# Xharlie/BtcDet

Hardware: AMD Instinct MI355X
Metric: scenes/s fwd+bwd KITTI-Car bs=2/GPU (BtcDet hot path) (higher is better)
Workload: dtype f32

## Files before the change

btcdet_amd/_lib.py:

```python
import ctypes
import os

import numpy as np
import torch

_HERE = os.path.dirname(os.path.abspath(__file__))
LIB_PATH = os.path.join(_HERE, "libbtcdet_hip.so")
_lib = None

c_i32p = ctypes.POINTER(ctypes.c_int32)
c_f32p = ctypes.POINTER(ctypes.c_float)
vp = ctypes.c_void_p
ci = ctypes.c_int
sz = ctypes.c_size_t

MODE_SUBM, MODE_CONV, MODE_TRANSPOSE = 0, 1, 2


class BtcHipError(RuntimeError):
    pass


class BtcOccConfig(ctypes.Structure):
    _fields_ = [("batch", ctypes.c_int32), ("grid", ctypes.c_int32 * 3), ("sphere_grid", ctypes.c_int32 * 3),
# ... 102 lines not shown
    "btc_revoxelize_fill": (ci, [vp, vp, ci, ci, ci, c_i32p, ci, ci, vp, vp, vp, vp, sz, vp]),
    "btc_pass_occ_vox_ws_bytes": (sz, [ctypes.POINTER(BtcPovConfig), ci, ci]),
    "btc_pass_occ_vox_count": (ci, [ctypes.POINTER(BtcPovConfig), vp, vp, vp, vp, vp, vp, ci, ci, ci, vp, vp, sz, vp]),
    "btc_pass_occ_vox_fill": (ci, [ctypes.POINTER(BtcPovConfig), vp, ci, ci, ci, ci, ci, ci, vp, vp, vp, vp, vp, vp, sz, vp]),
    "btc_pass_occ_vox_fill_i32": (ci, [ctypes.POINTER(BtcPovConfig), vp, ci, ci, ci, ci, ci, ci, vp, vp, vp, vp, vp, vp, vp, vp, sz, vp]),
    "btc_occ_loss_ws_bytes": (sz, []),
    "btc_occ_loss_fwd": (ci, [vp, vp, vp, vp, vp, vp, vp, vp, ci, ctypes.c_longlong, ctypes.c_float, ctypes.c_float, ctypes.c_float, vp, vp, vp,
                              sz, vp]),
    "btc_occ_loss_bwd": (ci, [vp, vp, vp, vp, vp, vp, vp, vp, ci, ctypes.c_longlong, ctypes.c_float, vp, vp, vp, vp, vp]),
    "btc_occ_loss_fwd_total": (ci, [vp, vp, vp, vp, vp, vp, vp, vp, ci, ctypes.c_longlong, ctypes.c_float, ctypes.c_float, ctypes.c_float, vp, vp,
                                    vp, sz, vp]),
    "btc_occ_loss_bwd_total": (ci, [vp, vp, vp, vp, vp, vp, vp, vp, ci, ctypes.c_longlong, ctypes.c_float, vp, vp, vp, vp, vp]),
    "btc_dense_split_fwd": (ci, [vp, vp, ci, ci, ci, vp, vp, vp, vp]),
    "btc_occ_prob": (ci, [vp, vp, ci, ctypes.c_longlong, vp, vp]),
    "btc_dense_split_bwd": (ci, [vp, vp, vp, ci, ci, ci, vp, vp, vp]),
    "btc_cat_pad_fwd": (ci, [vp, ci, vp, ci, ctypes.c_longlong, ci, ci, vp, vp]),
    "btc_cat_pad_bwd": (ci, [vp, ci, ctypes.c_longlong, ci, vp, ci, vp, ci, vp]),
    "btc_sumsq2_ws_bytes": (sz, []),
    "btc_sumsq2_fwd": (ci, [vp, ctypes.c_longlong, ci, ctypes.c_double, vp, ctypes.c_longlong, ci, ctypes.c_double, vp, vp, sz, vp]),
    "btc_sumsq2_bwd": (ci, [vp, ctypes.c_longlong, ci, ctypes.c_float, vp, vp, ctypes.c_longlong, ci, ctypes.c_float, vp, vp, vp]),
    "btc_bn_ws_bytes": (sz, [ci]),
    "btc_bn_relu_fwd": (ci, [vp, ci, ci, vp, vp, vp, vp, vp, ctypes.c_float, ctypes.c_float, ci, ci, vp, vp, vp, vp, sz, vp]),
    "btc_spin": (ci, [ci, vp]),
    "btc_bn_relu_bwd": (ci, [vp, vp, vp, ci, ci, vp, vp, vp, ci, ci, vp, vp, vp, vp, sz, vp]),
    "btc_bn_relu_fwd_bf16": (ci, [vp, ci, ci, vp, vp, vp, vp, vp, ctypes.c_float, ctypes.c_float, ci, ci, vp, vp, vp, vp, sz, vp]),
    "btc_bn_relu_bwd_bf16": (ci, [vp, vp, vp, ci, ci, vp, vp, vp, ci, ci, vp, vp, vp, vp, sz, vp]),
    "btc_ball_query": (ci, [vp, vp, vp, vp, ci, ci, ctypes.c_float, ctypes.c_float, ci, vp, vp]),
    "btc_group_points": (ci, [vp, vp, vp, vp, ci, ci, ci, ci, vp, vp]),
    "btc_group_points_grad": (ci, [vp, vp, vp, vp, ci, ci, ci, ci, ci, vp, vp]),
    "btc_furthest_point_sampling": (ci, [vp, ci, ci, ci, vp, vp, vp]),
    "btc_three_nn": (ci, [vp, vp, vp, vp, ci, ci, vp, vp, vp]),
    "btc_three_interpolate": (ci, [vp, vp, vp, ci, ci, vp, vp]),
    "btc_three_interpolate_grad": (ci, [vp, vp, vp, ci, ci, ci, vp, vp]),
    "btc_bn_fuse_ws_bytes": (sz, []),
    "btc_conv_bn_relu_fwd": (ci, [ci, vp, vp, vp, vp, vp, ci, ci, ci, ci, vp, vp, vp, vp, vp, vp, ctypes.c_float, ctypes.c_float, ci, vp, vp, vp, vp, sz, vp, vp]),
    "btc_conv_bn_relu_fwd_src": (ci, [ci, vp, ctypes.c_longlong, vp, vp, vp, vp, ci, ci, ci, ci, vp, vp, vp, vp, vp, vp, ctypes.c_float, ctypes.c_float, ci, vp, vp, vp, vp, sz, vp, vp]),
    "btc_col_sum": (ci, [vp, ci, ci, vp, vp, sz, vp]),
    "btc_col_sum_bf16": (ci, [vp, ci, ci, vp, vp, sz, vp]),
    "btc_occ_targets_ws_bytes": (sz, [ctypes.POINTER(BtcOccConfig)]),
    "btc_occ_backproject_lut": (ci, [ctypes.POINTER(BtcOccConfig), vp, vp]),
    "btc_occ_targets": (ci, [ctypes.POINTER(BtcOccConfig), vp, vp, vp, ci, ci, ci, vp, vp, vp, vp, ci, vp, vp,
                             ctypes.POINTER(BtcOccBuffers), vp, sz, vp]),
}

EXPORTED_SYMBOLS = tuple(_SIGS.keys())

_INFER_SIGS = {
    "btc_conv_bn_eval_fwd": (ci, [ci, vp, ctypes.c_longlong, vp, vp, vp, vp, ci, ci, ci, ci, vp, vp, vp, vp, ctypes.c_float, ci, vp, vp]),
    "btc_det_select_nms_ws_bytes": (sz, [ci, ci]),
    "btc_det_select_nms": (ci, [vp, vp, ci, ci, ci, ci, ci, ctypes.c_float, ctypes.c_float, ci, ci, ci, vp, vp, vp, vp, sz, vp]),
    "btc_det_finish": (ci, [vp, vp, ci, ci, ci, ci, ci, ci, vp, vp, vp, vp, ci, vp, ci, ci, vp, ci, ci, c_f32p, ci, vp, vp, vp, vp, vp, vp]),
    "btc_occ_metrics_ws_bytes": (sz, [ci, ci]),
    "btc_occ_metrics": (ci, [vp, vp, vp, vp, ctypes.c_longlong, vp, vp, vp, ctypes.c_longlong, vp, vp, ci, ci, ci, vp, vp, sz, vp]),
    "btc_kitti_overlaps": (ci, [vp, vp, vp, vp, vp, c_i32p, ci, vp, vp, vp]),
    "btc_kitti_match_tp": (ci, [vp, vp, vp, vp, vp, vp, vp, c_i32p, ci, ci, ci, ci, ci, ci, vp, vp, vp]),
    "btc_kitti_match_stats_ws_bytes": (sz, [ci, ci, ci, ci, ci]),
    "btc_kitti_match_stats": (ci, [vp, vp, vp, vp, vp, vp, vp, vp, vp, vp, vp, c_i32p, ci, ci, ci, ci, ci, ci, ci, vp, vp, vp, sz, vp]),
}

INFER_EXPORTED_SYMBOLS = tuple(_INFER_SIGS.keys())

_AUGMENT_SIGS = {
    "btc_augment_ws_bytes": (sz, [ci, ci, ci]),
    "btc_augment_batch": (ci, [vp, ci, ci, vp, ci, vp, vp, vp, ctypes.c_longlong, vp, vp, vp, vp, ci, ctypes.c_longlong, vp, vp,
                               ctypes.c_longlong, vp, vp, vp, vp, sz, vp]),
    "btc_world_transform": (ci, [vp, ci, ci, vp, ci, vp, vp, vp, vp]),
}

AUGMENT_EXPORTED_SYMBOLS = tuple(_AUGMENT_SIGS.keys())

_BESTMATCH_SIGS = {
    "btc_place_templates": (ci, [vp, ctypes.c_longlong, vp, vp, vp, vp, vp, ci, ci, vp, vp, ctypes.c_longlong, ci, vp, vp]),
}

BESTMATCH_EXPORTED_SYMBOLS = tuple(_BESTMATCH_SIGS.keys())

_FRAMES_SIGS = {
    "btc_fov_crop_ws_bytes": (sz, [ci, ci]),
    "btc_fov_crop": (ci, [vp, ci, ci, vp, ci, vp, ci, vp, vp, vp, vp, sz, vp]),
}

FRAMES_EXPORTED_SYMBOLS = tuple(_FRAMES_SIGS.keys())


def lib():
    global _lib
    if _lib is None:
        if not os.path.exists(LIB_PATH):
            raise BtcHipError(
                f"{LIB_PATH} not found: build it with `python -c 'import __graft_entry__ as g; g.build()'` "
                f"or `make -C btcdet_amd/csrc` (there is no CPU fallback for the hot path)")
        L = ctypes.CDLL(LIB_PATH)
        for name, (res, args) in (list(_SIGS.items()) + list(_INFER_SIGS.items()) + list(_AUGMENT_SIGS.items()) + list(_BESTMATCH_SIGS.items()) +
                                  list(_FRAMES_SIGS.items())):
            fn = getattr(L, name)
            fn.restype = res
            fn.argtypes = args
        for kv in filter(None, os.environ.get("BTC_TUNE", "").split(",")):
            k, v = kv.split("=")
            if L.btc_tune_set(int(k), int(v)) != 0:
                raise BtcHipError("BTC_TUNE: bad entry %r" % kv)
        _lib = L
    return _lib


_fast = False


def fast():
    global _fast
    if _fast is False:
        _fast = None
        if os.environ.get("BTC_FASTPATH", "1") != "0":
            try:
                lib()
                from . import _btcfast
                if _btcfast.abi_version() == lib().btc_version():
                    _fast = _btcfast
            except ImportError:
                _fast = None
    return _fast


def check(rc, what):
    if rc != 0:
        msg = lib().btc_last_error().decode("utf-8", "replace")
        raise BtcHipError(f"{what} failed (code {rc}): {msg}")


_raw_stream = torch._C._cuda_getCurrentRawStream
_cur_device = torch._C._cuda_getDevice


def stream_ptr():
    return _raw_stream(_cur_device())


def ptr(t):
    if t is None:
        return None
    if not (t.is_cuda and t.is_contiguous()):
        raise BtcHipError("expected a contiguous tensor on the GPU (HIP) device")
    return t.data_ptr()


_I3_CACHE = {}


def i3(v):
    if isinstance(v, (int, np.integer)):
        key = (int(v),) * 3
    else:
        key = tuple(int(x) for x in np.asarray(v).reshape(-1))
        if len(key) != 3:
            raise BtcHipError(f"expected 3 values, got {v!r}")
    a = _I3_CACHE.get(key)
    if a is None:
        a = np.ascontiguousarray(np.array(key, dtype=np.int32))
        a.setflags(write=False)
        a_ptr = a.ctypes.data_as(c_i32p)
        _I3_CACHE[key] = a
        _I3P_CACHE[id(a)] = (a, a_ptr)
    return a


_I3P_CACHE = {}


def i3p(a):
    hit = _I3P_CACHE.get(id(a))
    if hit is not None and hit[0] is a:
        return hit[1]
    return a.ctypes.data_as(c_i32p)


def f32p(a):
    return a.ctypes.data_as(c_f32p)
# ... 5 lines not shown
```

btcdet_amd/csrc/conv_apply_bf16.hip:

```cpp
#include "conv_tile.h"

namespace {

__device__ unsigned short g_zero_row_b[128];

constexpr int B_STAGES = 3;

template <int WR, int WC, int NTW, int KC, bool PAIR = false>
__global__ __launch_bounds__(64 * WR * WC) void conv_apply_b(const unsigned short* __restrict__ feat, const unsigned short* __restrict__ Wq,
                                                             const float* __restrict__ bias, const int32_t* __restrict__ nbr,
                                                             const int32_t* __restrict__ order, int n_rows, int K, int Cred, int Cres,
                                                             unsigned short* __restrict__ out, int flags, const BnFuse bn) {
  extern __shared__ __attribute__((aligned(16))) char smem[];
  constexpr int NW = WR * WC, THREADS = 64 * NW;
  constexpr int TM = 16 * WR, TN = 16 * NTW * WC;
  constexpr int UPR = KC / 8;
  constexpr int RPB = (128 / (KC * 2)) < 1 ? 1 : (128 / (KC * 2));
  constexpr int A_UNITS = TM * UPR, B_UNITS = TN * UPR;
  constexpr int NAI_TOTAL = (A_UNITS + 63) / 64, NAI = (NAI_TOTAL + NW - 1) / NW;
  constexpr int NBI_TOTAL = (B_UNITS + 63) / 64, NBI = (NBI_TOTAL + NW - 1) / NW;
  constexpr int NPI = NAI + NBI;
  constexpr int A_BYTES = (TM * KC * 2 + 1023) / 1024 * 1024;
  constexpr int B_BYTES = (TN * KC * 2 + 1023) / 1024 * 1024;
  constexpr int STAGE = A_BYTES + B_BYTES;
  char* ring = smem;
  APPLY_TAIL(ring + B_STAGES * STAGE, TM, K);

  const int tid = threadIdx.x, lane = tid & 63, wave = tid >> 6;
  const int wr = wave / WC, wc = wave % WC;
  const ApplyTile tile = apply_tile_prologue<TM, THREADS>(s_nbr, s_kact, s_nact, s_row, nbr, order, n_rows, K, flags, wr);
  const int bx = tile.bx, n0 = blockIdx.y * TN, n_act = tile.n_act;
  const unsigned long long wave_act = tile.wave_act;
  static_assert(!PAIR || KC == 64, "PAIR: two 32-channel offsets per 64-channel item");
  const int n_chunks = PAIR ? 1 : Cred / KC;
  const int n_items = PAIR ? (n_act + 1) >> 1 : n_act * n_chunks;

  f32x4 acc[NTW];
#pragma unroll
  for (int nt = 0; nt < NTW; ++nt) acc[nt] = (f32x4){0.f, 0.f, 0.f, 0.f};

  int iq = 0, ir = 0, cq = 0, cr = 0;
  auto issue = [&](int st) {
    const int k = s_kact[PAIR ? 2 * iq : iq];
    const int k1 = (PAIR && 2 * iq + 1 < n_act) ? s_kact[2 * iq + 1] : -1;
    const int cc = PAIR ? 0 : ir * KC;
    if (++ir == n_chunks) { ir = 0; ++iq; }
    char* As = ring + st * STAGE;
    char* Bs = As + A_BYTES;
#pragma unroll
    for (int t = 0; t < NAI; ++t) {
      const int ai = (wave + NW * t) % NAI_TOTAL;
      const int U = ai * 64 + lane;
      if (A_UNITS % 64 == 0 || U < A_UNITS) {
        const int rloc = U / UPR;
        const int u = (U % UPR) ^ ((rloc / RPB) & (UPR - 1));
        const int ku = (PAIR && (u & 4)) ? k1 : k;
        const int nb = ku >= 0 ? s_nbr[rloc * K + ku] : -1;
        const unsigned short* src = nb >= 0 ? feat + (size_t)nb * Cred + cc + (PAIR ? (u & 3) : u) * 8 : g_zero_row_b;
        glds16(src, As + ai * 1024);
      }
    }
    const unsigned short* Wk = Wq + ((size_t)k * Cres + n0) * Cred + cc;
    const unsigned short* Wk1 = PAIR ? Wq + ((size_t)(k1 >= 0 ? k1 : k) * Cres + n0) * Cred : Wk;
#pragma unroll
    for (int t = 0; t < NBI; ++t) {
      const int bi = (wave + NW * t) % NBI_TOTAL;
      const int U = bi * 64 + lane;
      if (B_UNITS % 64 == 0 || U < B_UNITS) {
        const int c = U / UPR;
        const int u = (U % UPR) ^ ((c / RPB) & (UPR - 1));
        glds16(((PAIR && (u & 4)) ? Wk1 : Wk) + (size_t)c * Cred + (PAIR ? (u & 3) : u) * 8, Bs + bi * 1024);
      }
    }
  };

  const int arow = lane & 15, kq = lane >> 4;
  if (n_items > 0) issue(0);
  if (n_items > 1) issue(1);
  int st = 0;
  for (int item = 0; item < n_items; ++item) {
    if (item + 1 < n_items) wait_vm<NPI>();
    else wait_vm<0>();
    __builtin_amdgcn_s_barrier();
    asm volatile("" ::: "memory");
    if (item + 2 < n_items) issue(st == 0 ? 2 : st - 1);
    const int k = s_kact[PAIR ? 2 * cq : cq];
    const int k2 = (PAIR && 2 * cq + 1 < n_act) ? s_kact[2 * cq + 1] : -1;
    if (++cr == n_chunks) { cr = 0; ++cq; }
    const bool act0 = (wave_act >> k) & 1ull, act1 = PAIR && k2 >= 0 && ((wave_act >> k2) & 1ull);
    if (act0 || act1) {
      const char* A = ring + st * STAGE + (wr * 16 + arow) * (KC * 2);
      const char* B = ring + st * STAGE + A_BYTES;
      const int aswz = ((wr * 16 + arow) / RPB) & (UPR - 1);
      constexpr int STEPS = KC / 32;
      bf16x8 a[STEPS], b[STEPS][NTW];
#pragma unroll
      for (int s = 0; s < STEPS; ++s) {
        const int q = s * 4 + kq;
        a[s] = *(const bf16x8*)(A + ((q ^ aswz) * 16));
#pragma unroll
        for (int nt = 0; nt < NTW; ++nt) {
          const int col = (wc * NTW + nt) * 16 + arow;
          b[s][nt] = *(const bf16x8*)(B + col * (KC * 2) + ((q ^ ((col / RPB) & (UPR - 1))) * 16));
        }
      }
#pragma unroll
      for (int s = 0; s < STEPS; ++s) {
        if (PAIR && !(s ? act1 : act0)) continue;
#pragma unroll
        for (int nt = 0; nt < NTW; ++nt)
          acc[nt] = __builtin_amdgcn_mfma_f32_16x16x32_bf16(a[s], b[s][nt], acc[nt], 0, 0, 0);
      }
    }
// ... 116 lines not shown
```

btcdet_amd/csrc/conv_apply_glds.hip:

```cpp
#include "conv_tile.h"

namespace {

__device__ float g_zero_row[64];

constexpr int G_STAGES_DEFAULT = 3;
constexpr int G_STAGES_MAX = 8;

__device__ __forceinline__ void transpose4(const f32x4 v, float& y0, float& y1, float& y2, float& y3) {
  unsigned x0 = __float_as_uint(v[0]), x1 = __float_as_uint(v[1]), x2 = __float_as_uint(v[2]), x3 = __float_as_uint(v[3]);
  auto a = __builtin_amdgcn_permlane32_swap(x0, x2, false, false);
  x0 = a[0]; x2 = a[1];
  auto b = __builtin_amdgcn_permlane32_swap(x1, x3, false, false);
  x1 = b[0]; x3 = b[1];
  auto c = __builtin_amdgcn_permlane16_swap(x0, x1, false, false);
  x0 = c[0]; x1 = c[1];
  auto d = __builtin_amdgcn_permlane16_swap(x2, x3, false, false);
  x2 = d[0]; x3 = d[1];
  y0 = __uint_as_float(x0); y1 = __uint_as_float(x1); y2 = __uint_as_float(x2); y3 = __uint_as_float(x3);
}

template <int WR, int WC, int NTW, bool TRANS_W, int KC, bool BF>
__global__ __launch_bounds__(64 * WR * WC) void conv_apply_g(const void* __restrict__ feat_, const float* __restrict__ W,
                                                             const float* __restrict__ bias, const int32_t* __restrict__ nbr,
                                                             const int32_t* __restrict__ order, int n_rows, int K, int Cred, int Cres,
                                                             void* __restrict__ out_, int flags, int dbg, const BnFuse bn) {
  extern __shared__ __attribute__((aligned(16))) char smem[];
  const int S = ((flags >> APPLY_STAGES_SHIFT) & 15) ? ((flags >> APPLY_STAGES_SHIFT) & 15) : G_STAGES_DEFAULT;
  constexpr int NW = WR * WC, THREADS = 64 * NW;
  constexpr int TM = 16 * WR, TN = 16 * NTW * WC, NG = NTW * WC;
  constexpr int ES = BF ? 2 : 4;
  constexpr int UPR = KC * ES / 16;
  constexpr int UPB = KC / 4;
  constexpr int RPB = (128 / (KC * ES)) < 1 ? 1 : (128 / (KC * ES));
  constexpr int A_UNITS = TM * UPR;
  constexpr int NAI_TOTAL = (A_UNITS + 63) / 64;
  constexpr int NAI = (NAI_TOTAL + NW - 1) / NW;
  constexpr int NBI_TOTAL = KC * TN / 256;
  constexpr int NBI = (NBI_TOTAL + NW - 1) / NW;
  constexpr int NPI = NAI + NBI;
  constexpr int A_BYTES = (TM * KC * ES + 1023) / 1024 * 1024;
  constexpr int STAGE = A_BYTES + KC * TN * 4;
  char* ring = smem;
  APPLY_TAIL(ring + S * STAGE, TM, K);
  const char* feat = (const char*)feat_;

  const int tid = threadIdx.x, lane = tid & 63, wave = tid >> 6;
  const int wr = wave / WC, wc = wave % WC;
  const ApplyTile tile = apply_tile_prologue<TM, THREADS>(s_nbr, s_kact, s_nact, s_row, nbr, order, n_rows, K, flags, wr);
  const int bx = tile.bx, n0 = blockIdx.y * TN, n_act = tile.n_act;
  const unsigned long long wave_act = tile.wave_act;
  const int n_chunks = Cred / KC;
  const int n_items = (dbg & 32) ? 0 : n_act * n_chunks;
  if (dbg & 16) return;

  f32x4 acc[NTW];
#pragma unroll
  for (int nt = 0; nt < NTW; ++nt) acc[nt] = (f32x4){0.f, 0.f, 0.f, 0.f};

  int iq = 0, ir = 0, cq = 0, cr = 0;
  auto issue = [&](int st) {
    const int k = s_kact[iq];
    const int cc = ir * KC;
    if (++ir == n_chunks) { ir = 0; ++iq; }
    char* As = ring + st * STAGE;
    float* Bs = (float*)(As + A_BYTES);
#pragma unroll
    for (int t = 0; t < NAI; ++t) {
      if (dbg & 8) break;
      const int ai = (wave + NW * t) % NAI_TOTAL;
      const int U = ai * 64 + lane;
      if (A_UNITS % 64 == 0 || U < A_UNITS) {
        const int rloc = U / UPR;
        const int u = (U % UPR) ^ ((rloc / RPB) & (UPR - 1));
        const int nb = s_nbr[rloc * K + k];
        const char* src = nb >= 0 ? feat + ((size_t)nb * Cred + cc) * ES + u * 16 : (const char*)g_zero_row;
        glds16(src, As + ai * 1024);
      }
    }
    const float* Wk = W + (size_t)k * Cred * Cres;
#pragma unroll
    for (int t = 0; t < NBI; ++t) {
      if (dbg & 4) break;
      const int ii = (wave + NW * t) % NBI_TOTAL;
      const int U = ii * 64 + lane;
      const float* src;
      if (!TRANS_W) {
        const int kr = U / (TN / 4), pu = U % (TN / 4);
        const int g = (NG >= 2) ? ((pu >> 2) ^ (kr & 1)) : (pu >> 2);
        src = Wk + (size_t)(cc + kr) * Cres + n0 + g * 16 + (pu & 3) * 4;
      } else {
        const int c = U / UPB, pu = U % UPB;
        const int ru = pu ^ (c & (UPB - 1));
        src = Wk + (size_t)(n0 + c) * Cred + cc + ru * 4;
      }
      glds16(src, Bs + ii * 256);
    }
  };

  const int arow = lane & 15, kq = lane >> 4;
#define WAIT_ITEMS(n) wait_vm<((n) * NPI > 63 ? 63 : (n) * NPI)>()
  for (int i = 0; i < S - 1 && i < n_items; ++i) issue(i);
  int st = 0;
  for (int item = 0; item < n_items; ++item) {
    const int left = n_items - 1 - item, fl = left < S - 2 ? left : S - 2;
    switch (fl) {
      case 0: wait_vm<0>(); break;
      case 1: WAIT_ITEMS(1); break;
      case 2: WAIT_ITEMS(2); break;
      case 3: WAIT_ITEMS(3); break;
      case 4: WAIT_ITEMS(4); break;
      case 5: WAIT_ITEMS(5); break;
      default: WAIT_ITEMS(6); break;
    }
#undef WAIT_ITEMS
    __builtin_amdgcn_s_barrier();
    asm volatile("" ::: "memory");
    if (item + S - 1 < n_items && !(dbg & 2)) issue(st == 0 ? S - 1 : st - 1);
    const int k = s_kact[cq];
    if (++cr == n_chunks) { cr = 0; ++cq; }
    if (((wave_act >> k) & 1ull) && !(dbg & 1)) {
      const char* A = ring + st * STAGE + (wr * 16 + arow) * (KC * ES);
      const float* B = (const float*)(ring + st * STAGE + A_BYTES);
      const int aswz = ((wr * 16 + arow) / RPB) & (UPR - 1);
      constexpr int Q = KC / 4;
      constexpr int G = (16 / NTW) < 1 ? 1 : ((16 / NTW) > Q ? Q : (16 / NTW));
      constexpr int NGRP = Q / G;
      float a[2][G], b[2][G][NTW];
      constexpr bool A128 = !BF && (G % 4 == 0);
      constexpr bool B128 = TRANS_W && (G % 4 == 0) && UPB >= 8 && NTW == 1;
      auto load_group = [&](int g, int buf) {
        if (A128) {
// ... 173 lines not shown
```

btcdet_amd/csrc/conv_apply_split.hip:

```cpp
#include "conv_tile.h"

namespace {

#define BTC_RSRC_RECORDS 0xFFFFFF00u
#define BTC_RSRC_ABSENT 0xFFFFFFF0u
__device__ __forceinline__ void blds16s(__amdgpu_buffer_rsrc_t rsrc, unsigned voffset, void* l) {
  __builtin_amdgcn_raw_ptr_buffer_load_lds(rsrc, (__attribute__((address_space(3))) void*)l, 16, voffset, 0, 0, 0);
}

template <int WR, int WC, int NTW, int KC, int S_STAGES, int LW, bool PAIR = false>
__global__ __launch_bounds__(64 * (WR * WC + LW)) void conv_apply_s(const float* __restrict__ feat, const unsigned short* __restrict__ Ws,
                                                             const float* __restrict__ bias, const int32_t* __restrict__ nbr,
                                                             const int32_t* __restrict__ order, int n_rows, int K, int Cred, int Cres,
                                                             float* __restrict__ out, int flags, const BnFuse bn) {
  extern __shared__ __attribute__((aligned(16))) char smem[];
  constexpr int NW = WR * WC, THREADS = 64 * (NW + LW);
  constexpr int NLD = LW ? LW : NW;
  constexpr int TM = 16 * WR, TN = 16 * NTW * WC;
  constexpr int UPA = KC / 4, UPB = KC / 8;
  constexpr int A_UNITS = TM * UPA, B_UNITS = 3 * TN * UPB;
  static_assert(A_UNITS % 64 == 0 && B_UNITS % 64 == 0, "whole DMA instructions");
  constexpr int NAI_TOTAL = A_UNITS / 64, NAI = (NAI_TOTAL + NLD - 1) / NLD;
  constexpr int NBI_TOTAL = B_UNITS / 64, NBI = (NBI_TOTAL + NLD - 1) / NLD;
  static_assert(LW == 0 || (NAI_TOTAL % LW == 0 && NBI_TOTAL % LW == 0), "the loader waves share the pieces evenly");
  constexpr int NPI = NAI + NBI;
  constexpr int A_BYTES = TM * KC * 4, P_BYTES = TN * KC * 2;
  constexpr int STAGE = A_BYTES + 3 * P_BYTES;
  char* ring = smem;
  APPLY_TAIL(ring + S_STAGES * STAGE, TM, K);

  const int tid = threadIdx.x, lane = tid & 63, wave = tid >> 6;
  const bool computes = LW == 0 || wave < NW, loads = LW == 0 || wave >= NW;
  const int wr = computes ? wave / WC : 0, wc = wave % WC;
  const int lid = LW ? wave - NW : wave;
  const int dbg = flags >> APPLY_DEBUG_SHIFT;
  const ApplyTile tile = apply_tile_prologue<TM, THREADS>(s_nbr, s_kact, s_nact, s_row, nbr, order, n_rows, K, flags, wr);
  const int bx = tile.bx, n0 = blockIdx.y * TN;
  const unsigned long long wave_act = tile.wave_act;
  const size_t plane = (size_t)K * Cred * Cres;
  const int n_act = __builtin_amdgcn_readfirstlane(tile.n_act);
  static_assert(!PAIR || KC == 64, "PAIR: two 32-channel offsets per 64-channel item");
  const int n_chunks = PAIR ? 1 : Cred / KC;
  const int n_pairs = PAIR ? (n_act + 1) >> 1 : n_act;
  const int n_all = n_pairs * n_chunks;
  const int i0 = (int)((long long)blockIdx.z * n_all / gridDim.z);
  const int n_items = (dbg & 32) ? i0 : (int)((long long)(blockIdx.z + 1) * n_all / gridDim.z);
  out += (size_t)blockIdx.z * n_rows * Cres;

  int iq = i0 / n_chunks, ir = i0 - iq * n_chunks;
  int cq = iq, cr = ir;
  const __amdgpu_buffer_rsrc_t rfeat = __builtin_amdgcn_make_buffer_rsrc((void*)feat, 0, BTC_RSRC_RECORDS, 0x00020000);
  const int kvec = lane < n_act ? s_kact[lane] : 0;
  int nbq[NAI];
  auto load_nbq = [&]() {
    if (PAIR) {
      const int k0 = __builtin_amdgcn_readlane(kvec, (2 * iq) & 63);
      const int k1 = (2 * iq + 1 < n_act) ? __builtin_amdgcn_readlane(kvec, (2 * iq + 1) & 63) : -1;
#pragma unroll
      for (int t = 0; t < NAI; ++t) {
        const int U = ((lid + NLD * t) % NAI_TOTAL) * 64 + lane;
        const int rloc = U / UPA;
        const int u = (U % UPA) ^ ((rloc ^ (rloc >> 3)) & (UPA - 1));
        const int k = (u & 8) ? k1 : k0;
        nbq[t] = k >= 0 ? s_nbr[rloc * K + k] : -1;
      }
      return;
    }
    const int k = __builtin_amdgcn_readlane(kvec, iq);
#pragma unroll
    for (int t = 0; t < NAI; ++t) {
      const int U = ((lid + NLD * t) % NAI_TOTAL) * 64 + lane;
      nbq[t] = s_nbr[(U / UPA) * K + k];
    }
  };
  if (loads) load_nbq();
  const __amdgpu_buffer_rsrc_t rw = __builtin_amdgcn_make_buffer_rsrc((void*)Ws, 0, BTC_RSRC_RECORDS, 0x00020000);
  static_assert(NLD % 2 == 0 && (TN * UPB) % 64 == 0 && 64 % UPB == 0, "one lane offset per issuing wave");
  const int w_c = lane / UPB;
  const int w_su = (lane % UPB) ^ (((w_c >> 1) + (UPB == 8 ? 4 * (lid & 1) : 0)) & (UPB - 1));
  const unsigned w_lane = (unsigned)(w_c * Cred + (PAIR ? (w_su & 3) : w_su) * 8) * 2u;
  auto issue = [&](int st) {
    const int k = __builtin_amdgcn_readlane(kvec, PAIR ? ((2 * iq) & 63) : iq);
    const int k1 = PAIR ? ((2 * iq + 1 < n_act) ? __builtin_amdgcn_readlane(kvec, (2 * iq + 1) & 63) : k) : k;
    const unsigned w_lane_i = PAIR ? w_lane + ((w_su & 4) ? (unsigned)((size_t)(k1 - k) * Cres * Cred) * 2u : 0u) : w_lane;
    const int cc = ir * KC;
    char* As = ring + st * STAGE;
    char* Bs = As + A_BYTES;
#pragma unroll
    for (int t = 0; t < NAI; ++t) {
      if (dbg & 8) break;
      const int ai = (lid + NLD * t) % NAI_TOTAL;
      const int U = ai * 64 + lane;
      const int rloc = U / UPA;
      const int u = (U % UPA) ^ ((rloc ^ (rloc >> 3)) & (UPA - 1));
      const int nb = nbq[t];
      blds16s(rfeat, nb >= 0 ? ((unsigned)nb * (unsigned)Cred + (unsigned)(PAIR ? (u & 7) * 4 : cc + u * 4)) * 4u : BTC_RSRC_ABSENT, As + ai * 1024);
    }
    const unsigned w_item = (unsigned)(((size_t)k * Cres + n0) * Cred + (PAIR ? 0 : cc)) * 2u;
#pragma unroll
    for (int t = 0; t < NBI; ++t) {
      if (dbg & 4) break;
      const int bi = (lid + NLD * t) % NBI_TOTAL;
      const int pl = (bi * 64) / (TN * UPB), c0 = ((bi * 64) % (TN * UPB)) / UPB;
      const unsigned w_piece = (unsigned)((size_t)pl * plane + (size_t)c0 * Cred) * 2u;
      __builtin_amdgcn_raw_ptr_buffer_load_lds(rw, (__attribute__((address_space(3))) void*)(Bs + bi * 1024), 16, w_lane_i, w_item + w_piece, 0, 0);
    }
    if (++ir == n_chunks) {
      ir = 0;
      ++iq;
      load_nbq();
    }
  };

  const int arow = lane & 15, kg = lane >> 4;
  static_assert((S_STAGES - 2) * NPI <= 63, "vmcnt is a 6-bit counter");
  float vals[NTW][4];
  bool valid[4];
  if (LW > 0 && wave >= NW) {
#pragma unroll
    for (int i = 0; i < S_STAGES - 1; ++i)
      if (i0 + i < n_items) issue(i);
    int st = 0;
    for (int item = i0; item < n_items; ++item) {
      const int left = n_items - 1 - item;
      if (S_STAGES >= 4 && left >= 2) wait_vm<(S_STAGES >= 4 ? 2 : 0) * NPI>();
      else if (S_STAGES >= 3 && left >= 1) wait_vm<(S_STAGES >= 3 ? 1 : 0) * NPI>();
      else wait_vm<0>();
      __builtin_amdgcn_s_barrier();
      asm volatile("" ::: "memory");
      if (item + S_STAGES - 1 < n_items && !(dbg & 2)) issue(st == 0 ? S_STAGES - 1 : st - 1);
// ... 34 lines not shown
        const char* B = ring + st * STAGE + A_BYTES;
        const int aswz = (r ^ (r >> 3)) & (UPA - 1);
        constexpr int STEPS = KC / 32;
        constexpr int GS = (NTW >= 4) ? 1 : STEPS;
#pragma unroll
        for (int g = 0; g < STEPS / GS; ++g) {
          f32x4 av[GS][2];
          bf16x8 bh[GS][NTW], bm[GS][NTW], bl[GS][NTW];
#pragma unroll
          for (int j = 0; j < GS; ++j) {
            const int u0 = 8 * (g * GS + j) + 2 * kg;
            av[j][0] = *(const f32x4*)(A + ((u0 ^ aswz) * 16));
            av[j][1] = *(const f32x4*)(A + (((u0 + 1) ^ aswz) * 16));
          }
#pragma unroll
          for (int j = 0; j < GS; ++j)
#pragma unroll
            for (int nt = 0; nt < NTW; ++nt) {
              const int col = (wc * NTW + nt) * 16 + arow;
              const char* bp = B + col * (KC * 2) + (((4 * (g * GS + j) + kg) ^ ((col >> 1) & (UPB - 1))) * 16);
              bh[j][nt] = *(const bf16x8*)bp;
              bm[j][nt] = *(const bf16x8*)(bp + P_BYTES);
              bl[j][nt] = *(const bf16x8*)(bp + 2 * P_BYTES);
            }
          __builtin_amdgcn_sched_barrier(0);
#pragma unroll
          for (int j = 0; j < GS; ++j) {
            if (PAIR && !((g * GS + j) ? act1 : act0)) continue;
            const f32x4 v0 = av[j][0], v1 = av[j][1];
            uint4 ah, am, al;
            btc_split3(v0[0], v0[1], ah.x, am.x, al.x);
            btc_split3(v0[2], v0[3], ah.y, am.y, al.y);
            btc_split3(v1[0], v1[1], ah.z, am.z, al.z);
            btc_split3(v1[2], v1[3], ah.w, am.w, al.w);
            const bf16x8 Ah = __builtin_bit_cast(bf16x8, ah), Am = __builtin_bit_cast(bf16x8, am), Al = __builtin_bit_cast(bf16x8, al);
#define S_MFMA(ACC, X, Y)                 \
    _Pragma("unroll") for (int nt = 0; nt < NTW; ++nt) ACC[nt] = __builtin_amdgcn_mfma_f32_16x16x32_bf16(X, Y[j][nt], ACC[nt], 0, 0, 0)
            S_MFMA(accs, Al, bh);
            S_MFMA(accs, Ah, bl);
            S_MFMA(accs, Am, bm);
            S_MFMA(accm, Am, bh);
            S_MFMA(accm, Ah, bm);
            S_MFMA(acc, Ah, bh);
#undef S_MFMA
          }
        }
      }
      st = (st == S_STAGES - 1) ? 0 : st + 1;
    }

    const bool ev = bn.ev_mean != nullptr;
#pragma unroll
    for (int nt = 0; nt < NTW; ++nt) {
      const int col = n0 + (wc * NTW + nt) * 16 + (lane & 15);
      const float bv0 = bias ? bias[col] : 0.f;
      BnEvalCol ec = {0.f, 0.f, 1.f, 0.f};
      if (ev) ec = bn_eval_col(bn, col);
#pragma unroll
      for (int r = 0; r < 4; ++r) {
        const int row = s_row[wr * 16 + kg * 4 + r];
        valid[r] = row >= 0;
        const float sum = acc[nt][r] + (accm[nt][r] + accs[nt][r]);
        float v = bias ? (sum + bv0) : sum;
        if (ev) v = bn_affine(v, ec.m, ec.rs, ec.g, ec.b, bn.ev_relu);
        if (row >= 0) out[(size_t)row * Cres + col] = v;
        vals[nt][r] = v;
      }
    }
  }
  if (bn.slots) {
    if (computes) bn_fuse_wave<NTW>(bn, vals, valid, n0 + wc * NTW * 16, (int)((bx * WR + wr) & (bn.nslots - 1)));
    bn_fuse_finish(bn, (int*)smem, (double*)(smem + 16));
  }
}

size_t lds_bytes_s(int tm, int tn, int kc, int K, int stages) {
  return (size_t)stages * ((size_t)tm * kc * 4 + (size_t)3 * tn * kc * 2) + apply_tail_bytes(tm, K);
}

template <int WR, int WC, int NTW, int KC, int S_STAGES, int LW = 0, bool PAIR = false>
int launch_s(const float* feat, const unsigned short* Ws, const float* bias, const int32_t* nbr, const int32_t* order, int n_rows, int K, int Cred,
             int Cres, float* out, int flags, hipStream_t stream, const BnFuse& bn, int zsplit) {
  constexpr int TM = 16 * WR, TN = 16 * NTW * WC;
  return apply_launch<conv_apply_s<WR, WC, NTW, KC, S_STAGES, LW, PAIR>>("conv_apply_s", dim3(btc_cdiv(n_rows, TM), Cres / TN, zsplit), 64 * (WR * WC + LW),
                                                                        lds_bytes_s(TM, TN, KC, K, S_STAGES), stream, feat, Ws, bias, nbr, order, n_rows, K,
                                                                        Cred, Cres, out, flags, bn);
}

__global__ __launch_bounds__(256) void split_reduce(const float* __restrict__ slabs, int Z, const float* __restrict__ bias, int n_rows, int Cres,
                                                    float* __restrict__ out, const BnFuse bn) {
  __shared__ int s_flag;
  const int lane = threadIdx.x & 63, wave = threadIdx.x >> 6;
  const int cq = lane & 15, rq = lane >> 4;
  const int col = blockIdx.y * 64 + cq * 4;
  const int row0 = (blockIdx.x * 4 + wave) * 16;
  const size_t slab = (size_t)n_rows * Cres;
  const f32x4 b = bias ? *(const f32x4*)(bias + col) : (f32x4){0.f, 0.f, 0.f, 0.f};
  double s1[4] = {0.0, 0.0, 0.0, 0.0}, s2[4] = {0.0, 0.0, 0.0, 0.0};
  const bool ev = bn.ev_mean != nullptr;
  BnEvalCol ec[4] = {};
  if (ev) {
#pragma unroll
    for (int e = 0; e < 4; ++e) ec[e] = bn_eval_col(bn, col + e);
  }
#pragma unroll
  for (int i = 0; i < 4; ++i) {
    const int row = row0 + i * 4 + rq;
    if (row < n_rows) {
      const float* p = slabs + (size_t)row * Cres + col;
      f32x4 v = *(const f32x4*)p;
      for (int z = 1; z < Z; ++z) v += *(const f32x4*)(p + z * slab);
      if (bias) v += b;
      if (ev) {
#pragma unroll
        for (int e = 0; e < 4; ++e) v[e] = bn_affine(v[e], ec[e].m, ec[e].rs, ec[e].g, ec[e].b, bn.ev_relu);
      }
      *(f32x4*)(out + (size_t)row * Cres + col) = v;
#pragma unroll
      for (int e = 0; e < 4; ++e) {
        s1[e] += (double)v[e];
        s2[e] += (double)v[e] * (double)v[e];
      }
    }
  }
  if (bn.slots) {
    const int slot = (int)((blockIdx.x * 4 + wave) & (bn.nslots - 1));
#pragma unroll
    for (int e = 0; e < 4; ++e) {
      s1[e] += __shfl_xor(s1[e], 16, 64);
      s2[e] += __shfl_xor(s2[e], 16, 64);
      s1[e] += __shfl_xor(s1[e], 32, 64);
      s2[e] += __shfl_xor(s2[e], 32, 64);
      if (lane < 16 && col + e < bn.C) {
        double* p = bn.slots + ((size_t)slot * 2) * BN_FUSE_CMAX + col + e;
        unsafeAtomicAdd(p, s1[e]);
        unsafeAtomicAdd(p + BN_FUSE_CMAX, s2[e]);
      }
    }
    bn_fuse_finish(bn, &s_flag);
  }
}

constexpr int SPLIT_MULTI_MAX = 32;
struct SplitTable {
  const float* W[SPLIT_MULTI_MAX];
  unsigned short* w_s[SPLIT_MULTI_MAX];
  unsigned short* wt_s[SPLIT_MULTI_MAX];
  int K[SPLIT_MULTI_MAX], Cin[SPLIT_MULTI_MAX], Cout[SPLIT_MULTI_MAX], first_block[SPLIT_MULTI_MAX + 1];
  int n;
};

__global__ __launch_bounds__(256) void weights_split3_multi(const SplitTable t) {
  int s = 0;
  while (s + 1 < t.n && (int)blockIdx.x >= t.first_block[s + 1]) ++s;
  const long long e = (long long)((int)blockIdx.x - t.first_block[s]) * 256 + threadIdx.x;
  const int Cin = t.Cin[s], Cout = t.Cout[s];
  const long long per = (long long)Cin * Cout, n = (long long)t.K[s] * per;
  if (e >= n) return;
  const BtcSplit3 x = btc_split3(t.W[s][e]);
  const unsigned short p[3] = {(unsigned short)(x.hi >> 16), (unsigned short)(x.mid >> 16), (unsigned short)(x.lo >> 16)};
  const int k = (int)(e / per);
  const int rem = (int)(e - (long long)k * per);
  const int ci = rem / Cout, co = rem - ci * Cout;
  const long long et = (long long)k * per + (long long)co * Cin + ci;
#pragma unroll
  for (int j = 0; j < 3; ++j) {
    t.w_s[s][j * n + e] = p[j];
    t.wt_s[s][j * n + et] = p[j];
  }
}

}

extern "C" int btc_weights_split3_multi(const float* const* W, void* const* w_split, void* const* wt_split, const int32_t* K, const int32_t* Cin,
                                        const int32_t* Cout, int n, void* stream) {
  BTC_CHECK_ARG(n >= 0, "btc_weights_split3_multi: bad count");
  for (int base = 0; base < n; base += SPLIT_MULTI_MAX) {
    SplitTable t;
    t.n = n - base < SPLIT_MULTI_MAX ? n - base : SPLIT_MULTI_MAX;
    int blocks = 0;
    for (int i = 0; i < t.n; ++i) {
      BTC_CHECK_ARG(K[base + i] >= 1 && Cin[base + i] >= 1 && Cout[base + i] >= 1, "btc_weights_split3_multi: bad sizes");
      t.W[i] = W[base + i];
      t.w_s[i] = (unsigned short*)w_split[base + i];
      t.wt_s[i] = (unsigned short*)wt_split[base + i];
      t.K[i] = K[base + i]; t.Cin[i] = Cin[base + i]; t.Cout[i] = Cout[base + i];
      t.first_block[i] = blocks;
      blocks += (int)btc_cdiv((long long)K[base + i] * Cin[base + i] * Cout[base + i], 256);
    }
    t.first_block[t.n] = blocks;
    if (blocks > 0) weights_split3_multi<<<blocks, 256, 0, (hipStream_t)stream>>>(t);
    BTC_LAUNCH_CHECK();
  }
  return BTC_OK;
}

extern "C" int btc_conv_split_supported(int K, int Cred, int Cres) {
  return K >= 1 && K <= 64 && Cred >= 32 && Cred % 32 == 0 && Cres >= 32 && Cres % 32 == 0;
}

static bool btc_split_pair_wanted(int K, int n_rows, int shape) { return K >= 8 && shape != 422 && n_rows >= 5000; }

extern "C" int btc_conv_split_wanted(int K, int Cred, int Cres, int n_rows) {
  return btc_tune_get(BTC_TUNE_SPLIT) != 1 && btc_conv_split_supported(K, Cred, Cres) &&
         n_rows >= ((Cred >= 128 || Cres >= 128) ? 2500 : (Cres % 64 == 0 ? (Cred >= 64 ? 2500 : 6000) : 20000));
}

int btc_apply_split(const float* src, const void* Ws_, const float* bias_, const int32_t* nbr, const int32_t* order, int n_rows, int K, int Cred,
                    int Cres, float* dst_, hipStream_t stream, int mirror, const BnFuse* bn_) {
  if (n_rows <= 0) return BTC_OK;
  const float* bias = bias_;
  float* dst = dst_;
  BTC_CHECK_ARG(btc_conv_split_supported(K, Cred, Cres), "conv_apply_s: needs K <= 64, Cred %% 32 == 0, Cres %% 64 == 0 (K=%d, %d -> %d)", K, Cred, Cres);
  const BnFuse bn = bn_ ? *bn_ : btc_bn_fuse_none();
  const unsigned short* Ws = (const unsigned short*)Ws_;
  const int flags = apply_flags(mirror) | (btc_tune_get(BTC_TUNE_APPLY_DEBUG) << APPLY_DEBUG_SHIFT);
  const int t_nt = btc_tune_get(BTC_TUNE_APPLY_NT);
  size_t scratch_bytes = 0;
  float* scratch = (float*)btc_scratch(stream, &scratch_bytes);
  const int t_z = btc_tune_get(BTC_TUNE_SPLIT_Z);
  const bool few = n_rows < 10000;
  if (scratch_bytes > BTC_SCRATCH_HEAD) {
    scratch = (float*)((char*)scratch + BTC_SCRATCH_HEAD);
    scratch_bytes -= BTC_SCRATCH_HEAD;
  } else {
    scratch = nullptr;
    scratch_bytes = 0;
  }
  const bool can_z = few && t_z != 1 && scratch_bytes >= (size_t)2 * n_rows * Cres * sizeof(float);
  int shape = (Cres % 128 == 0) ? ((!few || can_z || Cres >= 256) ? 424 : 222) : ((!few || can_z) ? 422 : 222);
  if (Cres % 64 != 0) shape = n_rows >= 100000 ? 412 : 812;
  if ((Cres % 128 != 0 && n_rows >= 5000 && n_rows < 22000) || (K <= 4 && n_rows < 22000)) shape = 412;
  if (Cres % 64 != 0 && Cred == 32 && K >= 8 && n_rows >= 5000 && btc_tune_get(BTC_TUNE_SPLIT_PAIR) != 1 && btc_tune_get(BTC_TUNE_APPLY_KC) != 32) shape = 412;
  if ((t_nt == 812 || t_nt == 412) && Cres % 32 == 0) shape = t_nt;
  if ((t_nt == 224 || t_nt == 424) && Cres % 128 == 0) shape = t_nt;
  if ((t_nt == 222 || t_nt == 422 || t_nt == 414 || t_nt == 814) && Cres % 64 == 0) shape = t_nt;
  if ((t_nt == 418 || t_nt == 818) && Cres % 128 == 0) shape = t_nt;
  const int t_kc = btc_tune_get(BTC_TUNE_APPLY_KC), t_st = btc_tune_get(BTC_TUNE_APPLY_STAGES);
  int kc = (Cred % 64 == 0 && (shape % 10 == 4 || n_rows < 22000) && shape % 100 != 12) ? 64 : 32;
  if (t_kc == 32 || (t_kc == 64 && Cred % 64 == 0)) kc = t_kc;
  if (shape % 100 == 12) kc = (Cred % 64 == 0 && t_kc != 32) ? 64 : 32;
  if (shape == 818) kc = 32;
  const int t_pair = btc_tune_get(BTC_TUNE_SPLIT_PAIR);
  const bool pair = Cred == 32 && t_pair != 1 && t_kc != 32 && (shape == 412 || shape == 812 || shape == 422) && (t_pair == 2 || btc_split_pair_wanted(K, n_rows, shape));
  if (pair) kc = 64;
  int stages = t_st ? t_st : 3;
  if (kc == 64) stages = (t_st == 3 && shape == 422) ? 3 : 2;
  const int items = K * (Cred / kc);
  int Z = 1;
  if (can_z && shape % 100 != 12 && items >= 12) {
    Z = t_z > 1 ? t_z : ((Cres % 128 == 0 || n_rows < 4000) ? 4 : 2);
    if (Z > items / 6) Z = items / 6;
    while (Z > 1 && (size_t)Z * n_rows * Cres * sizeof(float) > scratch_bytes) --Z;
    if (Z > 1) dst = scratch;
  }
  const BnFuse bn_kernel = Z > 1 ? btc_bn_fuse_none() : bn;
  if (Z > 1) bias = nullptr;
#define S_ARGS src, Ws, bias, nbr, order, n_rows, K, Cred, Cres, dst, flags, stream, bn_kernel, Z
  int rc = BTC_EINVAL;
  const int t_lw = btc_tune_get(BTC_TUNE_SPLIT_LOADERS);
  int lw = t_lw == 2 ? 2 : (t_lw == 4 ? 4 : (t_lw == 1 ? 0 : (kc == 64 ? 4 : (shape == 412 ? 2 : 0))));
  {
    const int tm = (shape / 100) * 16, tn = 16 * ((shape / 10) % 10) * (shape % 10);
    if (lw == 4 && ((tm * kc / 256) % 4 != 0 || (3 * tn * kc / 512) % 4 != 0)) lw = 2;
  }
#define S_CASE(code, WR_, WC_, NTW_, KC_, ST_)                                                                          \
  case code:                                                                                                           \
    if constexpr ((16 * WR_ * KC_ / 256) % 4 == 0 && (3 * 16 * NTW_ * WC_ * KC_ / 512) % 4 == 0) {                       \
      if (lw == 4) { rc = launch_s<WR_, WC_, NTW_, KC_, ST_, 4>(S_ARGS); break; }                                       \
    }                                                                                                                  \
    rc = lw ? launch_s<WR_, WC_, NTW_, KC_, ST_, 2>(S_ARGS) : launch_s<WR_, WC_, NTW_, KC_, ST_, 0>(S_ARGS);            \
    break
#define S_PAIR(code, WR_, WC_, NTW_)                                                                                     \
  case code:                                                                                                           \
    rc = lw == 4 ? launch_s<WR_, WC_, NTW_, 64, 2, 4, true>(S_ARGS)                                                      \
// ... 55 lines not shown
```

btcdet_amd/csrc/conv_tile.h:

```cpp
#pragma once
#include <type_traits>

#include "btc_common.h"
#include "bn_fuse.h"

typedef __bf16 bf16x8 __attribute__((ext_vector_type(8)));

constexpr int APPLY_XCD = 1;
constexpr int APPLY_MIRROR = 2;
constexpr int APPLY_STAGES_SHIFT = 4;
constexpr int APPLY_DEBUG_SHIFT = 8;
inline int apply_flags(int mirror) { return (btc_tune_get(BTC_TUNE_APPLY_XCD) == 2 ? APPLY_XCD : 0) | (mirror ? APPLY_MIRROR : 0); }

inline size_t apply_tail_bytes(int tm, int K) { return (size_t)(tm * K + K + 1 + tm) * sizeof(int32_t); }
#define APPLY_TAIL(base, TM_, K_)              \
  int32_t* s_nbr = (int32_t*)(base);           \
  int32_t* s_kact = s_nbr + (TM_) * (K_);      \
  int32_t* s_nact = s_kact + (K_);             \
  int32_t* s_row = s_nact + 1

struct ApplyTile {
  int bx, row0, n_act;
  unsigned long long wave_act;
};

template <int TM, int THREADS>
__device__ __forceinline__ ApplyTile apply_tile_prologue(int32_t* s_nbr, int32_t* s_kact, int32_t* s_nact, int32_t* s_row, const int32_t* __restrict__ nbr,
                                                         const int32_t* __restrict__ order, int n_rows, int K, int flags, int wr) {
  const int tid = threadIdx.x, lane = tid & 63, wave = tid >> 6;
  const int mirror = (flags & APPLY_MIRROR) ? 1 : 0;
  int bx = blockIdx.x;
  if (flags & APPLY_XCD) {
    const int nb = gridDim.x, per = nb >> 3, main = per << 3;
    if (bx < main) bx = (bx & 7) * per + (bx >> 3);
  }
  const int row0 = bx * TM;
  for (int e = tid; e < K; e += THREADS) s_kact[e] = 0;
  for (int e = tid; e < TM; e += THREADS) s_row[e] = (row0 + e < n_rows) ? (order ? order[row0 + e] : row0 + e) : -1;
  __syncthreads();
  for (int e = tid; e < TM * K; e += THREADS) {
    const int rloc = e / K, kk = e - rloc * K;
    const int gr = s_row[rloc];
    const int v = gr >= 0 ? nbr[(long long)gr * K + (mirror ? K - 1 - kk : kk)] : -1;
    s_nbr[e] = v;
    if (v >= 0) s_kact[kk] = 1;
  }
  __syncthreads();
  unsigned long long wave_act;
  {
    bool any = false;
    if (lane < K)
      for (int r = 0; r < 16; ++r) any |= s_nbr[(wr * 16 + r) * K + lane] >= 0;
    wave_act = __ballot(any);
  }
  const int kflag = (lane < K) ? s_kact[lane] : 0;
  __syncthreads();
  if (wave == 0) {
    const unsigned long long m = __ballot(kflag != 0);
    if (kflag) s_kact[__popcll(m & ((1ull << lane) - 1ull))] = lane;
    if (lane == 0) *s_nact = __popcll(m);
  }
  __syncthreads();
  return {bx, row0, *s_nact, wave_act};
}

template <int NTW, bool COLS = false, typename OUT>
__device__ __forceinline__ void apply_tile_epilogue(const f32x4 (&sum)[NTW], const int (&rows)[4], int col0, const float* __restrict__ bias, int Cres,
                                                    OUT* __restrict__ out, const BnFuse& bn, bool ev, float (&vals)[NTW][4], bool (&valid)[4]) {
#pragma unroll
  for (int r = 0; r < 4; ++r) valid[r] = rows[r] >= 0;
#pragma unroll
  for (int nt = 0; nt < NTW; ++nt) {
    const int col = col0 + nt * 16 + (threadIdx.x & 15);
    const float bv0 = (bias && (!COLS || col < Cres)) ? bias[col] : 0.f;
    BnEvalCol ec = {0.f, 0.f, 1.f, 0.f};
    if (ev) ec = bn_eval_col(bn, col);
#pragma unroll
    for (int r = 0; r < 4; ++r) {
      float v = bias ? (sum[nt][r] + bv0) : sum[nt][r];
      if (sizeof(OUT) == 2) {
        unsigned short h = btc_f32_to_bf16(v);
        if (ev) h = btc_f32_to_bf16(bn_affine(btc_bf16_to_f32(h), ec.m, ec.rs, ec.g, ec.b, bn.ev_relu));
        if (rows[r] >= 0) ((unsigned short*)out)[(size_t)rows[r] * Cres + col] = h;
        v = btc_bf16_to_f32(h);
      } else {
        if (ev) v = bn_affine(v, ec.m, ec.rs, ec.g, ec.b, bn.ev_relu);
        if ((!COLS || col < Cres) && rows[r] >= 0) ((float*)out)[(size_t)rows[r] * Cres + col] = v;
      }
      vals[nt][r] = v;
    }
  }
}

__device__ __forceinline__ void glds16(const void* g, void* l) {
  __builtin_amdgcn_global_load_lds((const __attribute__((address_space(1))) void*)g, (__attribute__((address_space(3))) void*)l, 16, 0, 0);
}
template <int N>
__device__ __forceinline__ void wait_vm() {
  asm volatile("s_waitcnt vmcnt(%0)" ::"n"(N) : "memory");
}

__device__ __forceinline__ float btc_split_rest(float x) { return x - __uint_as_float(__float_as_uint(x) & 0xFFFF0000u); }
struct BtcSplit3 { unsigned hi, mid, lo; };
__device__ __forceinline__ BtcSplit3 btc_split3(float x) {
  const float x1 = btc_split_rest(x), x2 = btc_split_rest(x1);
  return {__float_as_uint(x), __float_as_uint(x1), __float_as_uint(x2)};
}
__device__ __forceinline__ void btc_split3(float a, float b, unsigned& hi, unsigned& mid, unsigned& lo) {
  hi = __builtin_amdgcn_perm(__float_as_uint(b), __float_as_uint(a), 0x07060302u);
  const float a1 = btc_split_rest(a), b1 = btc_split_rest(b);
  mid = __builtin_amdgcn_perm(__float_as_uint(b1), __float_as_uint(a1), 0x07060302u);
  const float a2 = btc_split_rest(a1), b2 = btc_split_rest(b1);
  lo = __builtin_amdgcn_perm(__float_as_uint(b2), __float_as_uint(a2), 0x07060302u);
}
// ... 12 lines not shown
```

Measured before the change: 592.0.

## Remap split-conv workgroups so each XCD owns contiguous weight slices

Adds a slice-aware 1D grid mapping for the split-precision sparse conv apply kernel. Each of the 8 XCD-strided workgroup groups is assigned a contiguous range of (column block, z-split) slices, so every XCD touches only a subset of the weight planes, and the mapping is enabled automatically when the split weights exceed a 4 MB per-XCD L2 estimate. The intent is to cut L2 misses and HBM weight traffic for large layers. The cost is integer decode work per block, possible load imbalance across slices, and a host table export used for checking.

After: 594.1, median of 4. No clear change (+0.3%).

```diff
diff --git a/btcdet_amd/_lib.py b/btcdet_amd/_lib.py
--- a/btcdet_amd/_lib.py
+++ b/btcdet_amd/_lib.py
@@ -208,6 +208,12 @@
 
 FRAMES_EXPORTED_SYMBOLS = tuple(_FRAMES_SIGS.keys())
 
+_DISPATCH_SIGS = {
+    "btc_apply_slice_table": (ci, [ci, ci, ci, vp]),
+}
+
+DISPATCH_EXPORTED_SYMBOLS = tuple(_DISPATCH_SIGS.keys())
+
 
 def lib():
     global _lib
@@ -218,7 +224,7 @@
                 f"or `make -C btcdet_amd/csrc` (there is no CPU fallback for the hot path)")
         L = ctypes.CDLL(LIB_PATH)
         for name, (res, args) in (list(_SIGS.items()) + list(_INFER_SIGS.items()) + list(_AUGMENT_SIGS.items()) + list(_BESTMATCH_SIGS.items()) +
-                                  list(_FRAMES_SIGS.items())):
+                                  list(_FRAMES_SIGS.items()) + list(_DISPATCH_SIGS.items())):
             fn = getattr(L, name)
             fn.restype = res
             fn.argtypes = args
diff --git a/btcdet_amd/csrc/conv_apply_bf16.hip b/btcdet_amd/csrc/conv_apply_bf16.hip
--- a/btcdet_amd/csrc/conv_apply_bf16.hip
+++ b/btcdet_amd/csrc/conv_apply_bf16.hip
@@ -28,7 +28,7 @@
 
   const int tid = threadIdx.x, lane = tid & 63, wave = tid >> 6;
   const int wr = wave / WC, wc = wave % WC;
-  const ApplyTile tile = apply_tile_prologue<TM, THREADS>(s_nbr, s_kact, s_nact, s_row, nbr, order, n_rows, K, flags, wr);
+  const ApplyTile tile = apply_tile_prologue<TM, THREADS>(s_nbr, s_kact, s_nact, s_row, nbr, order, n_rows, K, flags, wr, blockIdx.x);
   const int bx = tile.bx, n0 = blockIdx.y * TN, n_act = tile.n_act;
   const unsigned long long wave_act = tile.wave_act;
   static_assert(!PAIR || KC == 64, "PAIR: two 32-channel offsets per 64-channel item");
diff --git a/btcdet_amd/csrc/conv_apply_glds.hip b/btcdet_amd/csrc/conv_apply_glds.hip
--- a/btcdet_amd/csrc/conv_apply_glds.hip
+++ b/btcdet_amd/csrc/conv_apply_glds.hip
@@ -47,7 +47,7 @@
 
   const int tid = threadIdx.x, lane = tid & 63, wave = tid >> 6;
   const int wr = wave / WC, wc = wave % WC;
-  const ApplyTile tile = apply_tile_prologue<TM, THREADS>(s_nbr, s_kact, s_nact, s_row, nbr, order, n_rows, K, flags, wr);
+  const ApplyTile tile = apply_tile_prologue<TM, THREADS>(s_nbr, s_kact, s_nact, s_row, nbr, order, n_rows, K, flags, wr, blockIdx.x);
   const int bx = tile.bx, n0 = blockIdx.y * TN, n_act = tile.n_act;
   const unsigned long long wave_act = tile.wave_act;
   const int n_chunks = Cred / KC;
diff --git a/btcdet_amd/csrc/conv_apply_split.hip b/btcdet_amd/csrc/conv_apply_split.hip
--- a/btcdet_amd/csrc/conv_apply_split.hip
+++ b/btcdet_amd/csrc/conv_apply_split.hip
@@ -1,4 +1,5 @@
 #include "conv_tile.h"
+#include "../../include/btcdet_hip_dispatch.h"
 
 namespace {
 
@@ -12,7 +13,7 @@
 __global__ __launch_bounds__(64 * (WR * WC + LW)) void conv_apply_s(const float* __restrict__ feat, const unsigned short* __restrict__ Ws,
                                                              const float* __restrict__ bias, const int32_t* __restrict__ nbr,
                                                              const int32_t* __restrict__ order, int n_rows, int K, int Cred, int Cres,
-                                                             float* __restrict__ out, int flags, const BnFuse bn) {
+                                                             float* __restrict__ out, int flags, const BnFuse bn, int zs) {
   extern __shared__ __attribute__((aligned(16))) char smem[];
   constexpr int NW = WR * WC, THREADS = 64 * (NW + LW);
   constexpr int NLD = LW ? LW : NW;
@@ -34,8 +35,13 @@
   const int wr = computes ? wave / WC : 0, wc = wave % WC;
   const int lid = LW ? wave - NW : wave;
   const int dbg = flags >> APPLY_DEBUG_SHIFT;
-  const ApplyTile tile = apply_tile_prologue<TM, THREADS>(s_nbr, s_kact, s_nact, s_row, nbr, order, n_rows, K, flags, wr);
-  const int bx = tile.bx, n0 = blockIdx.y * TN;
+  int bx0 = blockIdx.x, by = blockIdx.y, bz = blockIdx.z, nz = gridDim.z;
+  if (flags & APPLY_SLICE) {
+    const ApplySlice m = apply_slice_map(blockIdx.x, (unsigned)(n_rows + TM - 1) / TM, (unsigned)Cres / TN, (unsigned)zs);
+    bx0 = m.tile; by = m.y; bz = m.z; nz = zs;
+  }
+  const ApplyTile tile = apply_tile_prologue<TM, THREADS>(s_nbr, s_kact, s_nact, s_row, nbr, order, n_rows, K, flags, wr, bx0);
+  const int bx = tile.bx, n0 = by * TN;
   const unsigned long long wave_act = tile.wave_act;
   const size_t plane = (size_t)K * Cred * Cres;
   const int n_act = __builtin_amdgcn_readfirstlane(tile.n_act);
@@ -43,9 +49,9 @@
   const int n_chunks = PAIR ? 1 : Cred / KC;
   const int n_pairs = PAIR ? (n_act + 1) >> 1 : n_act;
   const int n_all = n_pairs * n_chunks;
-  const int i0 = (int)((long long)blockIdx.z * n_all / gridDim.z);
-  const int n_items = (dbg & 32) ? i0 : (int)((long long)(blockIdx.z + 1) * n_all / gridDim.z);
-  out += (size_t)blockIdx.z * n_rows * Cres;
+  const int i0 = (int)((long long)bz * n_all / nz);
+  const int n_items = (dbg & 32) ? i0 : (int)((long long)(bz + 1) * n_all / nz);
+  out += (size_t)bz * n_rows * Cres;
 
   int iq = i0 / n_chunks, ir = i0 - iq * n_chunks;
   int cq = iq, cr = ir;
@@ -246,9 +252,11 @@
 int launch_s(const float* feat, const unsigned short* Ws, const float* bias, const int32_t* nbr, const int32_t* order, int n_rows, int K, int Cred,
              int Cres, float* out, int flags, hipStream_t stream, const BnFuse& bn, int zsplit) {
   constexpr int TM = 16 * WR, TN = 16 * NTW * WC;
-  return apply_launch<conv_apply_s<WR, WC, NTW, KC, S_STAGES, LW, PAIR>>("conv_apply_s", dim3(btc_cdiv(n_rows, TM), Cres / TN, zsplit), 64 * (WR * WC + LW),
-                                                                        lds_bytes_s(TM, TN, KC, K, S_STAGES), stream, feat, Ws, bias, nbr, order, n_rows, K,
-                                                                        Cred, Cres, out, flags, bn);
+  const int X = (int)btc_cdiv(n_rows, TM), Y = Cres / TN, S = Y * zsplit;
+  if (apply_slice_wanted(K, Cred, Cres, S) && (long long)X * S * S < (1LL << 31)) flags = (flags & ~APPLY_XCD) | APPLY_SLICE;
+  return apply_launch<conv_apply_s<WR, WC, NTW, KC, S_STAGES, LW, PAIR>>("conv_apply_s", (flags & APPLY_SLICE) ? dim3(X * S) : dim3(X, Y, zsplit),
+                                                                        64 * (WR * WC + LW), lds_bytes_s(TM, TN, KC, K, S_STAGES), stream, feat, Ws, bias, nbr,
+                                                                        order, n_rows, K, Cred, Cres, out, flags, bn, zsplit);
 }
 
 __global__ __launch_bounds__(256) void split_reduce(const float* __restrict__ slabs, int Z, const float* __restrict__ bias, int n_rows, int Cres,
@@ -355,6 +363,18 @@
     t.first_block[t.n] = blocks;
     if (blocks > 0) weights_split3_multi<<<blocks, 256, 0, (hipStream_t)stream>>>(t);
     BTC_LAUNCH_CHECK();
+  }
+  return BTC_OK;
+}
+
+extern "C" int btc_apply_slice_table(int tiles, int col_blocks, int z_slices, int32_t* h_tile_y_z) {
+  BTC_CHECK_ARG(h_tile_y_z != nullptr, "btc_apply_slice_table: missing h_tile_y_z");
+  BTC_CHECK_ARG(tiles >= 1 && col_blocks >= 1 && z_slices >= 1, "btc_apply_slice_table: need tiles, col_blocks, z_slices >= 1");
+  const long long S = (long long)col_blocks * z_slices, N = S * tiles;
+  BTC_CHECK_ARG(N * S < (1LL << 31), "btc_apply_slice_table: %lld workgroups in %lld slices are past the 32-bit decode", N, S);
+  for (long long id = 0; id < N; ++id) {
+    const ApplySlice m = apply_slice_map((unsigned)id, (unsigned)tiles, (unsigned)col_blocks, (unsigned)z_slices);
+    h_tile_y_z[3 * id] = m.tile; h_tile_y_z[3 * id + 1] = m.y; h_tile_y_z[3 * id + 2] = m.z;
   }
   return BTC_OK;
 }
diff --git a/btcdet_amd/csrc/conv_tile.h b/btcdet_amd/csrc/conv_tile.h
--- a/btcdet_amd/csrc/conv_tile.h
+++ b/btcdet_amd/csrc/conv_tile.h
@@ -8,9 +8,31 @@
 
 constexpr int APPLY_XCD = 1;
 constexpr int APPLY_MIRROR = 2;
+constexpr int APPLY_SLICE = 4;
 constexpr int APPLY_STAGES_SHIFT = 4;
 constexpr int APPLY_DEBUG_SHIFT = 8;
 inline int apply_flags(int mirror) { return (btc_tune_get(BTC_TUNE_APPLY_XCD) == 2 ? APPLY_XCD : 0) | (mirror ? APPLY_MIRROR : 0); }
+
+struct ApplySlice { int tile, y, z; };
+__host__ __device__ inline ApplySlice apply_slice_map(unsigned id, unsigned X, unsigned Y, unsigned Z) {
+  const unsigned S = Y * Z, N = X * S, R = N >> 3, M = R << 3;
+  unsigned s, tile;
+  if (id < M) {
+    const unsigned p = (id & 7u) * R + (id >> 3);
+    s = ((p + 1u) * S - 1u) / M;
+    tile = p - s * M / S;
+  } else {
+    const unsigned t = id - M, T = N - M;
+    s = t * S / T;
+    tile = X + t - ((s + 1u) * T + S - 1u) / S;
+  }
+  return {(int)tile, (int)(s % Y), (int)(s / Y)};
+}
+constexpr size_t XCD_L2_BYTES = (size_t)4 << 20;
+inline bool apply_slice_wanted(int K, int Cred, int Cres, int slices) {
+  const int t = btc_tune_get(BTC_TUNE_APPLY_XCD);
+  return t == 3 || (t == 0 && slices > 1 && (size_t)6 * K * Cred * Cres > XCD_L2_BYTES);
+}
 
 inline size_t apply_tail_bytes(int tm, int K) { return (size_t)(tm * K + K + 1 + tm) * sizeof(int32_t); }
 #define APPLY_TAIL(base, TM_, K_)              \
@@ -26,10 +48,9 @@
 
 template <int TM, int THREADS>
 __device__ __forceinline__ ApplyTile apply_tile_prologue(int32_t* s_nbr, int32_t* s_kact, int32_t* s_nact, int32_t* s_row, const int32_t* __restrict__ nbr,
-                                                         const int32_t* __restrict__ order, int n_rows, int K, int flags, int wr) {
+                                                         const int32_t* __restrict__ order, int n_rows, int K, int flags, int wr, int bx) {
   const int tid = threadIdx.x, lane = tid & 63, wave = tid >> 6;
   const int mirror = (flags & APPLY_MIRROR) ? 1 : 0;
-  int bx = blockIdx.x;
   if (flags & APPLY_XCD) {
     const int nb = gridDim.x, per = nb >> 3, main = per << 3;
     if (bx < main) bx = (bx & 7) * per + (bx >> 3);
diff --git a/include/btcdet_hip_dispatch.h b/include/btcdet_hip_dispatch.h
--- /dev/null
+++ b/include/btcdet_hip_dispatch.h
@@ -0,0 +1,17 @@
+#ifndef BTCDET_HIP_DISPATCH_H
+#define BTCDET_HIP_DISPATCH_H
+
+#include <stdint.h>
+
+#include "btcdet_hip.h"
+
+#ifdef __cplusplus
+extern "C" {
+#endif
+
+int btc_apply_slice_table(int tiles, int col_blocks, int z_slices, int32_t* h_tile_y_z);
+
+#ifdef __cplusplus
+}
+#endif
+#endif
```
